# avik-pal/RegNeuralDE.jl

Hardware: AMD Instinct MI355X
Metric: training-step samples/sec + mean NFE, MNIST Neural ODE bs=512 (higher is better)
Workload: dtype f32; 1 GPU; MNIST NODE regularized (error_est), Tsit5 reltol=abstol=1.4e-8, batch 512 per GPU, 1xMI355X per rank; step = loss fwd + reverse pass through the solver + InvDecay/Momentum update; the weights train during the timed steps (mean_nfe drifts with --steps: value_fixed_weights of --full is the stationary companion); global_batch=512, parallelism=single

## Files before the change

### regneuralde.jl_amd/csrc/rnde_reverse.hip

```cpp
#include "rnde_node.h"
#include "rnde_wgradx.h"

static rnde_status chain_bwd_run(rnde_node* h, const float* u_bar_dev, const float* saveval_bar_host, float* x_bar_dev,
                                 float* p_bar_dev, float* tspan_bar_host, hipStream_t s, bool sync = true, float* tspan_bar_dev = nullptr);
static rnde_status bwd_run(rnde_node* h, const float* u_bar_dev, const float* saveval_bar_host, float* x_bar_dev,
                           float* p_bar_dev, float* tspan_bar_host, hipStream_t s, bool sync = true, float* tspan_bar_dev = nullptr);


extern "C" rnde_status rnde_node_backward_async(rnde_node* h, const float* u_bar_dev, const float* saveval_bar_host, float* x_bar_dev,
                                                float* p_bar_dev, float* tspan_bar_dev, void* stream) {
    if (!h) return RNDE_ERR_BAD_ARG;
    if (!h->have_tape) { h->err = "no recorded forward"; return RNDE_ERR_NO_TAPE; }
    if (h->engine == 3) return chain_bwd_run(h, u_bar_dev, saveval_bar_host, x_bar_dev, p_bar_dev, nullptr, (hipStream_t)stream, false, tspan_bar_dev);
    return bwd_run(h, u_bar_dev, saveval_bar_host, x_bar_dev, p_bar_dev, nullptr, (hipStream_t)stream, false, tspan_bar_dev);
}

extern "C" rnde_status rnde_node_backward(rnde_node* h, const float* u_bar_dev, const float* saveval_bar_host,
                                          float* x_bar_dev, float* p_bar_dev, float* tspan_bar_host, void* stream) {
    if (!h) return RNDE_ERR_BAD_ARG;
    if (!h->have_tape) { h->err = "no recorded forward"; return RNDE_ERR_NO_TAPE; }
    if (h->engine == 3) return chain_bwd_run(h, u_bar_dev, saveval_bar_host, x_bar_dev, p_bar_dev, tspan_bar_host, (hipStream_t)stream);
    return bwd_run(h, u_bar_dev, saveval_bar_host, x_bar_dev, p_bar_dev, tspan_bar_host, (hipStream_t)stream);
}
extern "C" rnde_status rnde_node_backward_host(rnde_node* h, const float* u_bar, const float* saveval_bar, float* x_bar,
                                               float* p_bar, float* tspan_bar) {
    if (!h) return RNDE_ERR_BAD_ARG;
    float *ub = nullptr, *xb = nullptr, *pb = nullptr;
    const size_t nb = (size_t)h->D * h->B * 4;
    HIPCHK(h, hipMalloc((void**)&ub, nb)); HIPCHK(h, hipMalloc((void**)&xb, nb)); HIPCHK(h, hipMalloc((void**)&pb, (size_t)h->P * 4));
    HIPCHK(h, hipMemcpy(ub, u_bar, nb, hipMemcpyHostToDevice));
    rnde_status st = rnde_node_backward(h, ub, saveval_bar, xb, pb, tspan_bar, nullptr);
    if (st == RNDE_OK) { hipMemcpy(x_bar, xb, nb, hipMemcpyDeviceToHost); hipMemcpy(p_bar, pb, (size_t)h->P * 4, hipMemcpyDeviceToHost); }
    hipFree(ub); hipFree(xb); hipFree(pb);
    return st;
}

static rnde_status bwd_prepare(rnde_node* h) {
    BwdBuffers& b = h->bw;
    if (b.ready) return RNDE_OK;
    const size_t A = (size_t)h->D * h->Bpad_max, HB = (size_t)h->H * h->Bpad_max;
    const int cap = h->cfg.max_attempts;
    HIPCHK(h, hipMalloc((void**)&b.U, A * 4)); HIPCHK(h, hipMalloc((void**)&b.K1, A * 4)); HIPCHK(h, hipMalloc((void**)&b.UB1, A * 4));
    HIPCHK(h, hipMalloc((void**)&b.zi2, 2 * A * 4)); HIPCHK(h, hipMalloc((void**)&b.zi1, 2 * HB * 4));
    HIPCHK(h, hipMalloc((void**)&b.svb_att, (size_t)cap * 4));
    HIPCHK(h, hipMalloc((void**)&b.bstate, 2 * sizeof(BState) + 64)); HIPCHK(h, hipMalloc((void**)&b.ibstate, 2 * sizeof(IBState)));
    HIPCHK(h, hipMalloc((void**)&b.bpart, (size_t)(2 * h->nwg_max + 256) * 4 * 4)); HIPCHK(h, hipMalloc((void**)&b.ipart, (size_t)2 * h->nwg_max * 4 * 4));
    HIPCHK(h, hipMalloc((void**)&b.tspan_out, 2 * 4));
    const size_t nev = (size_t)6 * cap + 2;
    const size_t desc_blob = 2 * nev * sizeof(EvalDesc) + (size_t)cap * 4 + 64;
    HIPCHK(h, hipMalloc((void**)&b.ev1, desc_blob)); HIPCHK(h, hipMalloc((void**)&b.ev2, nev * sizeof(EvalDesc)));
    HIPCHK(h, hipHostMalloc((void**)&b.h_ev1, desc_blob)); HIPCHK(h, hipHostMalloc((void**)&b.h_ev2, nev * sizeof(EvalDesc)));
    HIPCHK(h, hipHostMalloc((void**)&b.h_svb, (size_t)cap * 4));
    const size_t seg = std::max((size_t)h->H * (h->D + 2), (size_t)h->D * (h->H + 2));
    b.slab_floats = seg * 256;
    HIPCHK(h, hipMalloc((void**)&b.slab, 2 * b.slab_floats * 4));
    HIPCHK(h, hipMalloc((void**)&b.slab_r, 2 * 16 * seg * 4));
    if (!h->wstream) {
        int prio_least = 0, prio_greatest = 0;
        (void)hipDeviceGetStreamPriorityRange(&prio_least, &prio_greatest);
        HIPCHK(h, hipStreamCreateWithPriority(&h->wstream, hipStreamNonBlocking, prio_least));
        h->wevents.resize(66);
        for (auto& e : h->wevents) HIPCHK(h, hipEventCreateWithFlags(&e, hipEventDisableTiming));
    }
    if (h->engine == 2) {
        HIPCHK(h, hipMalloc((void**)&b.UTB, A * 4)); HIPCHK(h, hipMalloc((void**)&b.UNB, A * 4)); HIPCHK(h, hipMalloc((void**)&b.UPB0, A * 4));
        HIPCHK(h, hipMalloc((void**)&b.GB, 15 * A * 4));
    }
    b.ready = true;
    return RNDE_OK;
}

static bool wgrad3_ok(int M, int Nx) {
    const bool tall = M >= Nx;
    const int wide = tall ? M : Nx + 2, narrow = tall ? Nx + 2 : M;
    return getenv("RNDE_WGRAD_LEGACY") == nullptr && getenv("RNDE_WGRAD_V2") == nullptr && M % 4 == 0 && Nx % 4 == 0 && wide > 656 &&
           wide <= 800 && narrow <= 112;
}
static rnde_status launch_wgrad_part(rnde_node* h, const EvalDesc* ev, int n_evals, int per_chunk, int M, int Nx, int Bpad,
                                     float* slab, int* chunk_cursor, hipStream_t s, int max_chunks = 0) {
    if (n_evals <= 0) return RNDE_OK;
    const int mtiles = (M + 31) / 32, ntiles = (Nx + 2 + 31) / 32;
    const bool tall = M >= Nx;
    const int MB = tall ? 2 : 4, NB = tall ? 4 : 2;
    const int blocks = ((mtiles + MB - 1) / MB) * ((ntiles + NB - 1) / NB);
    const long long len = (long long)M * (Nx + 2);
    const int chunks = (n_evals + per_chunk - 1) / per_chunk;
    float* dst = slab + (size_t)(*chunk_cursor) * len;
    static const bool legacy = getenv("RNDE_WGRAD_LEGACY") != nullptr;
    const bool fits = tall ? (Nx + 2 <= 128) : (M <= 128);
    if (wgrad3_ok(M, Nx)) {
        const int total_steps = n_evals * ((Bpad + 31) / 32);
        static const int target_chunks = getenv("RNDE_WGRAD3_CHUNKS") ? atoi(getenv("RNDE_WGRAD3_CHUNKS")) : 128;
        int sc = std::max(1, std::min({max_chunks > 0 ? max_chunks : target_chunks, total_steps, 256}));
        const int steps_per_chunk = (total_steps + sc - 1) / sc;
        sc = (total_steps + steps_per_chunk - 1) / steps_per_chunk;
        if ((size_t)(*chunk_cursor + sc) * (size_t)len > h->bw.slab_floats) { h->err = "weight-gradient slab overflow"; return RNDE_ERR_BAD_ARG; }
        const bool x3_off = getenv("RNDE_X3_WGRAD_OFF") != nullptr;
        const bool x3_half = getenv("RNDE_X3_WGRAD_HALF") != nullptr;
        const int TT4 = ((tall ? M : Nx + 2) + 15) / 16;
        if (h->x3_packed && !x3_off && !x3_half && TT4 >= 28 && TT4 <= 52) {
            static const int target4 = getenv("RNDE_WGRAD4_CHUNKS") ? atoi(getenv("RNDE_WGRAD4_CHUNKS")) : 64;
            int sc4 = std::max(1, std::min({max_chunks > 0 ? max_chunks / 2 : target4, total_steps, 256}));
            const int spc4 = (total_steps + sc4 - 1) / sc4;
            sc4 = (total_steps + spc4 - 1) / spc4;
            if ((size_t)(*chunk_cursor + sc4) * (size_t)len > h->bw.slab_floats) { h->err = "weight-gradient slab overflow"; return RNDE_ERR_BAD_ARG; }
            static DeviceOnce attr4;
            if (attr4.need()) {
                HIPCHK(h, hipFuncSetAttribute((const void*)rnde_wgrad4x_kernel<true>, hipFuncAttributeMaxDynamicSharedMemorySize, (int)kWx4LdsBytes));
                HIPCHK(h, hipFuncSetAttribute((const void*)rnde_wgrad4x_kernel<false>, hipFuncAttributeMaxDynamicSharedMemorySize, (int)kWx4LdsBytes));
                attr4.done();
            }
            const dim3 g4(32 * ((sc4 + 7) / 8));
            if (tall) hipLaunchKernelGGL((rnde_wgrad4x_kernel<true>), g4, dim3(448), kWx4LdsBytes, s, ev, n_evals, spc4, sc4, M, Nx, Bpad, dst);
            else hipLaunchKernelGGL((rnde_wgrad4x_kernel<false>), g4, dim3(448), kWx4LdsBytes, s, ev, n_evals, spc4, sc4, M, Nx, Bpad, dst);
            HIPCHK(h, hipGetLastError());
            *chunk_cursor += sc4;
            return RNDE_OK;
        }
        if (h->x3_packed && !x3_off) {
            static DeviceOnce attrx;
            if (attrx.need()) {
                HIPCHK(h, hipFuncSetAttribute((const void*)rnde_wgrad3x_kernel<true>, hipFuncAttributeMaxDynamicSharedMemorySize, (int)kWxLdsBytes));
                HIPCHK(h, hipFuncSetAttribute((const void*)rnde_wgrad3x_kernel<false>, hipFuncAttributeMaxDynamicSharedMemorySize, (int)kWxLdsBytes));
                attrx.done();
            }
            if (tall) hipLaunchKernelGGL((rnde_wgrad3x_kernel<true>), dim3(2, sc), dim3(448), kWxLdsBytes, s, ev, n_evals, steps_per_chunk, M, Nx, Bpad, dst);
            else hipLaunchKernelGGL((rnde_wgrad3x_kernel<false>), dim3(2, sc), dim3(448), kWxLdsBytes, s, ev, n_evals, steps_per_chunk, M, Nx, Bpad, dst);
            HIPCHK(h, hipGetLastError());
            *chunk_cursor += sc;
            return RNDE_OK;
        }
        const size_t lds = (size_t)2 * 32 * (464 + 144) * sizeof(float);
        static DeviceOnce attr;
        if (attr.need()) {
            HIPCHK(h, hipFuncSetAttribute((const void*)rnde_wgrad3_kernel<true>, hipFuncAttributeMaxDynamicSharedMemorySize, (int)lds));
            HIPCHK(h, hipFuncSetAttribute((const void*)rnde_wgrad3_kernel<false>, hipFuncAttributeMaxDynamicSharedMemorySize, (int)lds));
            attr.done();
        }
        if (tall) hipLaunchKernelGGL((rnde_wgrad3_kernel<true>), dim3(2, sc), dim3(448), lds, s, ev, n_evals, steps_per_chunk, M, Nx, Bpad, dst);
        else hipLaunchKernelGGL((rnde_wgrad3_kernel<false>), dim3(2, sc), dim3(448), lds, s, ev, n_evals, steps_per_chunk, M, Nx, Bpad, dst);
        HIPCHK(h, hipGetLastError());
        *chunk_cursor += sc;
        return RNDE_OK;
    }
    if (!legacy && fits) {
        const int pblocks = tall ? (M + 127) / 128 : (Nx + 2 + 127) / 128;
        const int total_steps = n_evals * ((Bpad + 31) / 32);
        static const int target_wgs = getenv("RNDE_WGRAD_WGS") ? atoi(getenv("RNDE_WGRAD_WGS")) : 768;
        int sc = std::max(1, std::min({target_wgs / pblocks, total_steps, 256}));
        const int steps_per_chunk = (total_steps + sc - 1) / sc;
        sc = (total_steps + steps_per_chunk - 1) / steps_per_chunk;
        if ((size_t)(*chunk_cursor + sc) * (size_t)len > h->bw.slab_floats) { h->err = "weight-gradient slab overflow"; return RNDE_ERR_BAD_ARG; }
        if (tall) hipLaunchKernelGGL((rnde_wgrad2_kernel<true>), dim3(pblocks, sc), dim3(256), 0, s, ev, n_evals, steps_per_chunk, M, Nx, Bpad, dst);
        else hipLaunchKernelGGL((rnde_wgrad2_kernel<false>), dim3(pblocks, sc), dim3(256), 0, s, ev, n_evals, steps_per_chunk, M, Nx, Bpad, dst);
        HIPCHK(h, hipGetLastError());
        *chunk_cursor += sc;
        return RNDE_OK;
    } else {
        if ((size_t)(*chunk_cursor + chunks) * (size_t)len > h->bw.slab_floats) { h->err = "weight-gradient slab overflow"; return RNDE_ERR_BAD_ARG; }
        if (tall) hipLaunchKernelGGL((rnde_wgrad_kernel<2, 4>), dim3(blocks, chunks), dim3(64), 0, s, ev, n_evals, per_chunk, M, Nx, Bpad, dst);
        else hipLaunchKernelGGL((rnde_wgrad_kernel<4, 2>), dim3(blocks, chunks), dim3(64), 0, s, ev, n_evals, per_chunk, M, Nx, Bpad, dst);
    }
    HIPCHK(h, hipGetLastError());
    *chunk_cursor += chunks;
    return RNDE_OK;
}
static rnde_status launch_wgrad_reduce(rnde_node* h, const float* slab, int chunks, int M, int Nx, float* out, hipStream_t s) {
    const long long len = (long long)M * (Nx + 2);
    const int grid = (int)std::min<long long>((len + 255) / 256, 2048);
    if (chunks <= 16) {
        hipLaunchKernelGGL(rnde_wgrad_reduce, dim3(grid, 1), dim3(256), 0, s, slab, chunks, chunks, len, out);
    } else {
        const int per_group = (chunks + 15) / 16, groups = (chunks + per_group - 1) / per_group;
        hipLaunchKernelGGL(rnde_wgrad_reduce, dim3(grid, groups), dim3(256), 0, s, slab, chunks, per_group, len, h->bw.slab_r);
        hipLaunchKernelGGL(rnde_wgrad_reduce, dim3(grid, 1), dim3(256), 0, s, (const float*)h->bw.slab_r, groups, groups, len, out);
    }
    HIPCHK(h, hipGetLastError());
    return RNDE_OK;
}

static rnde_status bwd_run(rnde_node* h, const float* u_bar_dev, const float* saveval_bar_host, float* x_bar_dev,
                           float* p_bar_dev, float* tspan_bar_host, hipStream_t s, bool sync, float* tspan_bar_dev) {
    HIPCHK(h, hipSetDevice(h->cfg.device));
    rnde_status st = bwd_prepare(h);
    if (st != RNDE_OK) return st;
    BwdBuffers& b = h->bw;
    int n_att = h->n_att;
    const float svb_scale = h->couple ? (float)h->couple_world : 1.f;
    for (int i = 0; i < n_att; ++i)
        b.h_svb[i] = (saveval_bar_host && h->sv_index[i] >= 0) ? svb_scale * saveval_bar_host[h->sv_index[i]] : 0.f;
    const int ne_all = 2 + 6 * n_att;
    EvalDesc* const h_ev1 = b.h_ev1; EvalDesc* const h_ev2 = b.h_ev1 + ne_all; float* const h_svb_blob = (float*)(b.h_ev1 + 2 * (size_t)ne_all);
    EvalDesc* const d_ev1 = b.ev1;   EvalDesc* const d_ev2 = b.ev1 + ne_all;   float* const d_svb = (float*)(b.ev1 + 2 * (size_t)ne_all);
    memcpy(h_svb_blob, b.h_svb, (size_t)n_att * 4);
    BwdParams Q{};
    Q.F = make_params(h, h->xcopy, h->B, h->t0, h->t1, 1);
    Q.U = b.U; Q.K1 = b.K1; Q.UB1 = b.UB1; Q.zi2 = b.zi2; Q.zi1 = b.zi1; Q.svb_att = d_svb;
    Q.bstate = b.bstate; Q.ibstate = b.ibstate; Q.bpart = b.bpart; Q.ipart = b.ipart;
    Q.ubar = u_bar_dev; Q.xbar = x_bar_dev; Q.tspan_out = b.tspan_out;
    Q.n_att = n_att; Q.track_ctrl = h->cfg.track_ctrl; Q.track_initdt = h->cfg.track_initdt; Q.reg_kind = h->cfg.regularize;
    Q.bpart_n = Q.F.nwg;
    Q.tspan_scale = h->couple ? 1.f / (float)h->couple_world : 1.f;
#ifdef RNDE_DIAG
    if (getenv("RNDE_DIAG_BWD")) { if (!h->diag_buf) hipMalloc((void**)&h->diag_buf, 8192); hipMemset(h->diag_buf, 0, 512); Q.F.dbg_out = h->diag_buf; }
#endif
    Q.sv_T = (int)h->saveat.size();
    Q.sv_ubar0 = (!h->saveat.empty() && h->saveat[0] == h->t0) ? u_bar_dev : nullptr;
    if (!h->saveat.empty() && h->engine != 2) { h->err = "saveat reverse pass runs on the stage engine only"; return RNDE_ERR_BAD_ARG; }
    const long long A = (long long)h->D * Q.F.Bpad, HB = (long long)h->H * Q.F.Bpad;
    RecLayout L{A, HB};
    int ne = 2;
    h_ev2[0] = EvalDesc{b.zi2, h->h0, h->t0, 0};           h_ev1[0] = EvalDesc{b.zi1, h->xcopy, h->t0, 0};
    h_ev2[1] = EvalDesc{b.zi2 + A, h->h1, h->t0 + h->h_init->dt0, 0}; h_ev1[1] = EvalDesc{b.zi1 + HB, h->u1, h->t0 + h->h_init->dt0, 0};
    for (int n = 0; n < n_att; ++n) {
        const StepMeta& m = h->h_meta[n];
        const float* R = h->arena + (long long)m.rec * h->rec_stride;
        for (int sidx = 2; sidx <= 7; ++sidx) {
            const float ts = m.t + tsC(sidx - 1) * m.dt;
            h_ev2[ne] = EvalDesc{R + L.k(sidx), R + L.h(sidx), ts, 0};
            h_ev1[ne] = EvalDesc{R + L.z1(sidx), sidx < 7 ? R + L.g(sidx) : R + L.unew(), ts, 0};
            ++ne;
        }
    }
    HIPCHK(h, hipMemcpyAsync(b.ev1, b.h_ev1, 2 * (size_t)ne * sizeof(EvalDesc) + (size_t)n_att * 4, hipMemcpyHostToDevice, s));
    float* slab1 = b.slab;
    float* slab2w = b.slab + b.slab_floats;
    int cur1 = 0, cur2 = 0, evi = 0;
    const int per_chunk = std::max(1, (ne + 239) / 240);
    const int side_pct = h->wgrad_side_pct;
    const int sweep_cus = 8 * h->sR * ((Q.F.Bpad / 16 + 7) / 8);
    const bool side = h->engine == 2 && h->persist == 1 && side_pct > 0 && n_att >= 8 && sweep_cus <= 224 &&
                      wgrad3_ok(h->H, h->D) && wgrad3_ok(h->D, h->H);
    const int side_att = side ? std::min(n_att, n_att * side_pct / 100) : 0;
    const int group = std::max(4, (side_att + 5) / 6);
    bool used_side = false;
    auto wgrad_group = [&](int lo, int hi, bool on_side) -> rnde_status {
        if (hi <= lo) return RNDE_OK;
        hipStream_t ws = s;
        if (on_side) {
            hipEvent_t ev = h->wevents[evi++ % 64];
            HIPCHK(h, hipEventRecord(ev, s));
            HIPCHK(h, hipStreamWaitEvent(h->wstream, ev, 0));
            ws = h->wstream; used_side = true;
        }
        rnde_status r = launch_wgrad_part(h, d_ev1 + lo, hi - lo, per_chunk, h->H, h->D, h->B, slab1, &cur1, ws, on_side ? 16 : 0);
        if (r != RNDE_OK) return r;
        return launch_wgrad_part(h, d_ev2 + lo, hi - lo, per_chunk, h->D, h->H, h->B, slab2w, &cur2, ws, on_side ? 16 : 0);
    };
    int hi_att = n_att;
    hipError_t e;
    h->tev_bwd = false;
    if (h->timing) HIPCHK(h, hipEventRecord(h->tev[2], s));
    if (h->engine == 2) {
        if (!h->rev_packed) {
            HIPCHK(h, stage_pack(h, h->pcopy, h->spwBt, 2, h->sMT, h->sKHb, s));
            HIPCHK(h, stage_pack(h, h->pcopy, h->spwDt, 3, h->sHT, h->sMT, s));
        }
        h->rev_packed = false;
        BStageParams BQ{};
        BQ.B = Q; BQ.p = h->pcopy; BQ.pwBt = h->spwBt; BQ.pwDt = h->spwDt; BQ.slab = h->slab2; BQ.x3Bt = h->x3Bt; BQ.x3Dt = h->x3Dt;
        BQ.UTB = b.UTB; BQ.UNB = b.UNB; BQ.UPB0 = b.UPB0; BQ.GB = b.GB;
        BQ.EXK = b.GB + 6 * A; BQ.EXG = b.GB + 7 * A; BQ.SVW = b.GB + 8 * A;
        BQ.sv_t = h->saveat.empty() ? nullptr : h->sv_t_dev; BQ.sv_ubar = u_bar_dev; BQ.nsave = (int)h->saveat.size();
        BQ.MT = h->sMT; BQ.WT = h->sWT; BQ.R = h->sR; BQ.C = Q.F.Bpad / 16; BQ.HT = h->sHT; BQ.KHb = h->sKHb;
        double* const bsum = (double*)(b.bstate + 2);
        const bool pre_reduce = h->persist == 1 && Q.bpart_n >= 896 && !getenv("RNDE_NO_BPART_REDUCE");
        if (pre_reduce) BQ.B.bsum = bsum;
        const dim3 grid(BQ.R * BQ.C), blk(64 * BQ.WT);
        std::vector<int> sv_lo(n_att, 0), sv_hi(n_att, 0);
        if (!h->saveat.empty()) {
            int ns = (h->saveat[0] == h->t0) ? 1 : 0;
            for (int n = 0; n < n_att; ++n) {
                sv_lo[n] = ns;
                if (h->h_meta[n].flags & F_ACCEPT) {
                    const float tnew = h->h_meta[n].t + h->h_meta[n].dt;
                    while (ns < (int)h->saveat.size() && h->saveat[ns] <= tnew) ++ns;
                }
                sv_hi[n] = ns;
            }
        }
        auto eig_coefs = [&](int n, float& c1, float& c2) {
            c1 = 0.f; c2 = 0.f;
            const StepMeta& mm = h->h_meta[n];
            const bool eg_ok = !(mm.eigen == 0.f || mm.eigen != mm.eigen);
            double eigb = 0.0;
            if (h->cfg.regularize == RNDE_REG_STIFF && eg_ok) eigb = (double)b.h_svb[n] * (mm.eigen > 0 ? 1.0 : -1.0) / 3.5068;
            if (h->cfg.regularize == RNDE_REG_ERR_STIFF && eg_ok) eigb = 0.1 * (double)b.h_svb[n] / 3.5068;
            if (h->cfg.regularize == RNDE_REG_STIFF_DT && eg_ok) eigb = (double)b.h_svb[n] * ((double)mm.eigen * (double)mm.dt > 0 ? 1.0 : -1.0) * (double)mm.dt;
            if (eigb != 0.0 && mm.n1 > 0.f && mm.n2 > 0.f) {
                c1 = (float)(eigb / ((double)mm.n2 * (double)mm.n1));
                c2 = (float)(-eigb * ((double)mm.n1 / (double)mm.n2) / ((double)mm.n2 * (double)mm.n2));
            }
        };
        for (int n = n_att - 1; n >= 0; --n) {
            float c1 = 0.f, c2 = 0.f;
            eig_coefs(n, c1, c2);
            const double qo = pow((double)h->h_meta[n].qold_in, (double)kBeta2);
            if (h->persist == 1) {
                PersistSync Y{h->tslab, h->pabort, h->pxcc, h->persist_spins};
                HIPCHK(h, slab_prepare(h, Q.F.Bpad, s));
                const dim3 pgrid(8 * BQ.R * ((BQ.C + 7) / 8));
                const bool fix = BQ.WT == 7 && BQ.HT == 7 && BQ.KHb == 7 && BQ.MT == 49 && BQ.R == 7 && h->D == 784 && h->H == 100 && !h->stage_generic;
                if (fix) {
                    const size_t flds = h->stage_lds + (size_t)(RNDE_BSTAGE_HDMA ? 1 : 0) * 6 * 7 * 2 * 1024;
                    static DeviceOnce attr;
                    if (attr.need()) {
                        HIPCHK(h, hipFuncSetAttribute((const void*)rnde_bstage_attempt_kernel<1, 1>, hipFuncAttributeMaxDynamicSharedMemorySize, 160 * 1024));
                        HIPCHK(h, hipFuncSetAttribute((const void*)rnde_bstage_attempt_kernel<0, 1>, hipFuncAttributeMaxDynamicSharedMemorySize, 160 * 1024));
                        attr.done();
                    }
                    const bool x3 = h->x3_packed && h->x3Bt && h->x3Dt && !getenv("RNDE_X3_REV_OFF");
                    if (x3) {
                        const size_t xlds = sizeof(float) * ((size_t)2 * kX3ImageFloats + 64) + (size_t)(RNDE_BSTAGE_HDMA ? 1 : 0) * 6 * 7 * 2 * 1024;
                        static DeviceOnce attr3;
                        if (attr3.need()) {
#define RNDE_X3_ATTR(A, E) HIPCHK(h, hipFuncSetAttribute((const void*)rnde_bstage_attempt_kernel<A, 1, 1, E>, hipFuncAttributeMaxDynamicSharedMemorySize, 160 * 1024));
                            RNDE_X3_ATTR(1, 0) RNDE_X3_ATTR(1, 1) RNDE_X3_ATTR(1, 2) RNDE_X3_ATTR(1, 3) RNDE_X3_ATTR(0, 0) RNDE_X3_ATTR(0, 1) RNDE_X3_ATTR(0, 2) RNDE_X3_ATTR(0, 3)
#undef RNDE_X3_ATTR
                            attr3.done();
                        }
                        const int ex = (h->saveat.empty() ? 0 : 1) | (h->cfg.regularize >= RNDE_REG_STIFF ? 2 : 0);
#define RNDE_X3_LAUNCH(A, E) hipLaunchKernelGGL((rnde_bstage_attempt_kernel<A, 1, 1, E>), pgrid, blk, xlds, s, BQ, n, h->h_meta[n], c1, c2, sv_lo[n], sv_hi[n], Y, qo, b.h_svb[n])
                        if (h->act2) { if (ex == 0) RNDE_X3_LAUNCH(1, 0); else if (ex == 1) RNDE_X3_LAUNCH(1, 1); else if (ex == 2) RNDE_X3_LAUNCH(1, 2); else RNDE_X3_LAUNCH(1, 3); }
                        else { if (ex == 0) RNDE_X3_LAUNCH(0, 0); else if (ex == 1) RNDE_X3_LAUNCH(0, 1); else if (ex == 2) RNDE_X3_LAUNCH(0, 2); else RNDE_X3_LAUNCH(0, 3); }
#undef RNDE_X3_LAUNCH
                    } else if (h->act2) hipLaunchKernelGGL((rnde_bstage_attempt_kernel<1, 1>), pgrid, blk, flds, s, BQ, n, h->h_meta[n], c1, c2, sv_lo[n], sv_hi[n], Y, qo, b.h_svb[n]);
                    else hipLaunchKernelGGL((rnde_bstage_attempt_kernel<0, 1>), pgrid, blk, flds, s, BQ, n, h->h_meta[n], c1, c2, sv_lo[n], sv_hi[n], Y, qo, b.h_svb[n]);
                } else if (h->act2) hipLaunchKernelGGL((rnde_bstage_attempt_kernel<1, 0>), pgrid, blk, h->stage_lds, s, BQ, n, h->h_meta[n], c1, c2, sv_lo[n], sv_hi[n], Y, qo, b.h_svb[n]);
                else hipLaunchKernelGGL((rnde_bstage_attempt_kernel<0, 0>), pgrid, blk, h->stage_lds, s, BQ, n, h->h_meta[n], c1, c2, sv_lo[n], sv_hi[n], Y, qo, b.h_svb[n]);
                if ((st = couple_sum(h, b.bpart + (size_t)(n & 1) * Q.bpart_n * 4, 4LL * Q.bpart_n, s)) != RNDE_OK) return st;
                if (pre_reduce && n > 0) hipLaunchKernelGGL(rnde_bpart_reduce_kernel, dim3(1), dim3(64), 0, s, Q, n, bsum);
                if (n >= n_att - side_att && (hi_att - n >= group || n == n_att - side_att)) {
                    st = wgrad_group(2 + 6 * n, 2 + 6 * hi_att, true);
                    if (st != RNDE_OK) return st;
                    hi_att = n;
                }
                continue;
            }
            if (h->act2) hipLaunchKernelGGL((rnde_bstage_kernel<1, BM_START>), grid, blk, h->stage_lds, s, BQ, n, 0, h->h_meta[n], c1, c2, sv_lo[n], sv_hi[n], qo);
            else hipLaunchKernelGGL((rnde_bstage_kernel<0, BM_START>), grid, blk, h->stage_lds, s, BQ, n, 0, h->h_meta[n], c1, c2, sv_lo[n], sv_hi[n], qo);
            for (int j = 6; j >= 1; --j) {
                if (h->act2) hipLaunchKernelGGL((rnde_bstage_kernel<1, BM_STAGE>), grid, blk, h->stage_lds, s, BQ, n, j, h->h_meta[n], c1, c2, sv_lo[n], sv_hi[n], qo);
                else hipLaunchKernelGGL((rnde_bstage_kernel<0, BM_STAGE>), grid, blk, h->stage_lds, s, BQ, n, j, h->h_meta[n], c1, c2, sv_lo[n], sv_hi[n], qo);
            }
            if ((st = couple_sum(h, b.bpart + (size_t)(n & 1) * Q.bpart_n * 4, 4LL * Q.bpart_n, s)) != RNDE_OK) return st;
        }
        HIPCHK(h, hipGetLastError());
        {
            if (h->act2) {
                hipLaunchKernelGGL((rnde_binit_stage_kernel<1, 0>), grid, blk, h->stage_lds, s, BQ);
                hipLaunchKernelGGL((rnde_binit_stage_kernel<1, 1>), grid, blk, h->stage_lds, s, BQ);
            } else {
                hipLaunchKernelGGL((rnde_binit_stage_kernel<0, 0>), grid, blk, h->stage_lds, s, BQ);
                hipLaunchKernelGGL((rnde_binit_stage_kernel<0, 1>), grid, blk, h->stage_lds, s, BQ);
            }
            if ((st = couple_sum(h, Q.ipart, 4LL * Q.F.nwg, s)) != RNDE_OK) return st;
            if (h->act2) {
                hipLaunchKernelGGL((rnde_binit_stage_kernel<1, 2>), grid, blk, h->stage_lds, s, BQ);
                hipLaunchKernelGGL((rnde_binit_stage_kernel<1, 3>), grid, blk, h->stage_lds, s, BQ);
            } else {
                hipLaunchKernelGGL((rnde_binit_stage_kernel<0, 2>), grid, blk, h->stage_lds, s, BQ);
                hipLaunchKernelGGL((rnde_binit_stage_kernel<0, 3>), grid, blk, h->stage_lds, s, BQ);
            }
            if ((st = couple_sum(h, Q.ipart + 4LL * Q.F.nwg, 4LL * Q.F.nwg, s)) != RNDE_OK) return st;
            hipLaunchKernelGGL(rnde_bfin_kernel, dim3(1), dim3(64), 0, s, Q);
            HIPCHK(h, hipGetLastError());
        }
    }
    if (h->timing) HIPCHK(h, hipEventRecord(h->tev[3], s));
    st = wgrad_group(0, 2 + 6 * hi_att, false);
    if (st != RNDE_OK) return st;
    if (used_side) {
        hipEvent_t ev = h->wevents[64];
        HIPCHK(h, hipEventRecord(ev, h->wstream));
        HIPCHK(h, hipStreamWaitEvent(s, ev, 0));
    }
    if (cur1 > 16 && cur2 > 16) {
        const long long len1 = (long long)h->H * (h->D + 2), len2 = (long long)h->D * (h->H + 2);
        const size_t seg_r = std::max((size_t)len1, (size_t)len2);
        float* r1 = b.slab_r; float* r2 = b.slab_r + 16 * seg_r;
        const int pg1 = (cur1 + 15) / 16, g1 = (cur1 + pg1 - 1) / pg1, pg2 = (cur2 + 15) / 16, g2 = (cur2 + pg2 - 1) / pg2;
        const int grid = (int)std::min<long long>((std::max(len1, len2) + 255) / 256, 2048);
        ReducePair A{{{slab1, r1, len1, cur1, pg1}, {slab2w, r2, len2, cur2, pg2}}};
        hipLaunchKernelGGL(rnde_wgrad_reduce_pair, dim3(grid, std::max(g1, g2), 2), dim3(256), 0, s, A);
        ReducePair Bp{{{r1, p_bar_dev, len1, g1, g1}, {r2, p_bar_dev + (size_t)h->H * (h->D + 2), len2, g2, g2}}};
        hipLaunchKernelGGL(rnde_wgrad_reduce_pair, dim3(grid, 1, 2), dim3(256), 0, s, Bp);
        HIPCHK(h, hipGetLastError());
    } else {
        st = launch_wgrad_reduce(h, slab1, cur1, h->H, h->D, p_bar_dev, s);
        if (st != RNDE_OK) return st;
        st = launch_wgrad_reduce(h, slab2w, cur2, h->D, h->H, p_bar_dev + (size_t)h->H * (h->D + 2), s);
        if (st != RNDE_OK) return st;
    }
    if (h->timing) { HIPCHK(h, hipEventRecord(h->tev[4], s)); h->tev_bwd = true; }
#ifdef RNDE_DIAG
    if (h->engine == 2 && h->persist == 1 && getenv("RNDE_DIAG_BWD")) {
        unsigned long long hst[64] = {0};
        hipStreamSynchronize(s);
        hipMemcpy(hst, h->diag_buf, sizeof(hst), hipMemcpyDeviceToHost);
        fprintf(stderr, "persistent reverse attempt (workgroup 0 thread 0, cycles): START %lld (entry->weights issued %lld, ->w1t %lld, ->array loads issued %lld, finish_attempt_scalars %lld, scalar chain %lld, vector part %lld), its phase D + put %lld\n", (long long)(hst[1]-hst[0]), (long long)(hst[43]-hst[0]), (long long)(hst[44]-hst[43]), (long long)(hst[40]-hst[44]), (long long)(hst[41]-hst[40]), (long long)(hst[42]-hst[41]), (long long)(hst[1]-hst[42]), (long long)(hst[2]-hst[1]));
        for (int st = 0; st < 6; ++st) { const unsigned long long* q = hst + 3 + 5 * st; const unsigned long long prev = st == 0 ? hst[2] : hst[7 + 5 * (st - 1)];
            fprintf(stderr, "  stage j=%d: poll %lld A %lld B %lld C %lld D+put %lld\n", 6 - st, (long long)(q[0]-prev), (long long)(q[1]-q[0]), (long long)(q[2]-q[1]), (long long)(q[3]-q[2]), st < 5 ? (long long)(q[4]-q[3]) : 0LL); }
        fprintf(stderr, "  total %lld cycles to the end of stage 1, END (reduction of the 21 partial sums) %lld; in START's vector part the wait for the record's k arrays %lld\n",
                (long long)(hst[34]-hst[0]), (long long)(hst[35]-hst[34]), (long long)(hst[45]-hst[42]));
    }
#endif
    if (!sync) {
        if (tspan_bar_dev) HIPCHK(h, hipMemcpyAsync(tspan_bar_dev, b.tspan_out, 8, hipMemcpyDeviceToDevice, s));
        h->have_tape = false;
        h->pending_bwd = (h->engine == 2 && h->persist == 1);
        return RNDE_OK;
    }
    HIPCHK(h, hipMemcpyAsync(h->h_scal, b.tspan_out, 8, hipMemcpyDeviceToHost, s));
    if (h->engine == 2) persist_check_enqueue(h, h->sR * (Q.F.Bpad / 16), s);
    HIPCHK(h, hipStreamSynchronize(s));
    if (h->couple && rnde_comm_health(h->couple) != RNDE_OK) { h->err = std::string("coupled controller: ") + rnde_comm_last_error(h->couple); return RNDE_ERR_HIP; }
    if (tspan_bar_host) { tspan_bar_host[0] = h->h_scal[0]; tspan_bar_host[1] = h->h_scal[1]; }
// ... 406 lines not shown
```

### regneuralde.jl_amd/csrc/rnde_wgradx.h

```cpp
#pragma once
#include "rnde_x3.h"

namespace rnde {

constexpr int kWxRowShorts = 40;
constexpr int kWxTallRows = 400, kWxNarrowRows = 112;
constexpr int kWxPlaneShortsT = kWxTallRows * kWxRowShorts, kWxPlaneShortsS = kWxNarrowRows * kWxRowShorts;
constexpr size_t kWxLdsBytes = (size_t)3 * (kWxPlaneShortsT + kWxPlaneShortsS) * 2;

template <bool TALL_IS_Z>
__global__ __launch_bounds__(448) void rnde_wgrad3x_kernel(const EvalDesc* __restrict__ evals, int n_evals, int per_chunk, int M, int Nx, int Bpad, float* __restrict__ slab) {
    constexpr int KC = 32;
    extern __shared__ __attribute__((aligned(16))) unsigned short wxs[];
    unsigned short* TP = wxs;
    unsigned short* SP = wxs + 3 * kWxPlaneShortsT;
    const int tid = threadIdx.x, lane = tid & 63, w = __builtin_amdgcn_readfirstlane(tid >> 6);
    const int mrow = lane & 15, kk = lane >> 4;
    const int TR = TALL_IS_Z ? M : Nx + 2, SR = TALL_IS_Z ? Nx + 2 : M;
    const int TRp = TALL_IS_Z ? M : Nx, SRp = TALL_IS_Z ? Nx : M;
    const int TT = (TR + 15) >> 4, T0 = (TT + 1) >> 1;
    const int half = blockIdx.x, chunk = blockIdx.y;
    const int tile_lo = half ? T0 : 0, tile_hi = half ? TT : T0, ntile = tile_hi - tile_lo;
    const int row_lo = 16 * tile_lo, nrow = 16 * ntile;
    const int steps_per_eval = (Bpad + KC - 1) / KC;
    const int s_lo = chunk * per_chunk, s_hi = min(n_evals * steps_per_eval, s_lo + per_chunk);
    const int total_steps = max(0, s_hi - s_lo);
    x3f4 acc[4][7];
#pragma unroll
    for (int i = 0; i < 4; ++i)
#pragma unroll
        for (int n = 0; n < 7; ++n) acc[i][n] = (x3f4){0.f, 0.f, 0.f, 0.f};
    const bool has3 = w + 21 < ntile;

    constexpr unsigned kNoSrc = 0x7FFFFF00u;
    int u_kind[5], u_dst[5];
    unsigned u_voff[5];
#pragma unroll
    for (int jj = 0; jj < 4; ++jj) {
        const int u = tid + 448 * jj;
        int kind = 0, dst = 0; unsigned voff = kNoSrc;
        if (u < 4 * nrow) {
            const int o = u / nrow, row = u - o * nrow, gr = row_lo + row;
            kind = gr < TRp ? 1 : (!TALL_IS_Z && gr == TRp ? 2 : (!TALL_IS_Z && gr == TRp + 1 ? 3 : 4));
            if (kind == 1) voff = 4u * (unsigned)(gr + 8 * o * TRp);
            dst = row * kWxRowShorts + 8 * o;
        }
        u_kind[jj] = kind; u_voff[jj] = voff; u_dst[jj] = dst;
    }
    {
        const int o = tid / kWxNarrowRows, row = tid - o * kWxNarrowRows;
        const int kind = row < SRp ? 1 : (TALL_IS_Z && row == SRp ? 2 : (TALL_IS_Z && row == SRp + 1 ? 3 : 4));
        u_kind[4] = kind; u_voff[4] = kind == 1 ? 4u * (unsigned)(row + 8 * o * SRp) : kNoSrc;
        u_dst[4] = 3 * kWxPlaneShortsT + row * kWxRowShorts + 8 * o;
    }
    int e_nx = s_lo / steps_per_eval, cs_nx = s_lo - e_nx * steps_per_eval;
    float stg[5][8];
    float stg_t = 0.f; int stg_ncols = 0;
    auto fetch = [&]() {
        const int e = e_nx, c0 = cs_nx * KC;
        if (++cs_nx == steps_per_eval) { cs_nx = 0; ++e_nx; }
        stg_t = evals[e].t;
        stg_ncols = min(KC, Bpad - c0);
        __amdgpu_buffer_rsrc_t rsT = __builtin_amdgcn_make_buffer_rsrc((void*)(TALL_IS_Z ? evals[e].Z : evals[e].X), 0, 4 * TRp * Bpad, 0x00020000);
        __amdgpu_buffer_rsrc_t rsS = __builtin_amdgcn_make_buffer_rsrc((void*)(TALL_IS_Z ? evals[e].X : evals[e].Z), 0, 4 * SRp * Bpad, 0x00020000);
#pragma unroll
        for (int jj = 0; jj < 5; ++jj) {
            const int cs = jj < 4 ? TRp : SRp;
#pragma unroll
            for (int j = 0; j < 8; ++j) {
                const unsigned off = u_voff[jj] + 4u * (unsigned)((c0 + j) * cs);
                stg[jj][j] = __builtin_bit_cast(float, __builtin_amdgcn_raw_buffer_load_b32(jj < 4 ? rsT : rsS, (int)off, 0, 2));
            }
        }
    };
    auto spill = [&]() {
#pragma unroll
        for (int jj = 0; jj < 5; ++jj) {
            const int kind = u_kind[jj];
            if (kind == 0) continue;
            const int o8 = u_dst[jj] % kWxRowShorts;
            float v[8];
#pragma unroll
            for (int j = 0; j < 8; ++j) v[j] = kind == 1 ? stg[jj][j] : ((kind == 2 || kind == 3) && o8 + j < stg_ncols ? (kind == 2 ? stg_t : 1.f) : 0.f);
            unsigned hi[4], mid[4], lo[4];
#pragma unroll
            for (int j = 0; j < 4; ++j) x3_split2(v[2 * j], v[2 * j + 1], hi[j], mid[j], lo[j]);
            unsigned short* d = wxs + u_dst[jj];
            const int ps = jj < 4 ? kWxPlaneShortsT : kWxPlaneShortsS;
            *(x3u4*)d = (x3u4){hi[0], hi[1], hi[2], hi[3]};
            *(x3u4*)(d + ps) = (x3u4){mid[0], mid[1], mid[2], mid[3]};
            *(x3u4*)(d + 2 * ps) = (x3u4){lo[0], lo[1], lo[2], lo[3]};
        }
    };
    auto fragT = [&](int tile, int pl) { return *(const x3u4*)(TP + pl * kWxPlaneShortsT + (16 * tile + mrow) * kWxRowShorts + 8 * kk); };
    auto fragS = [&](int tile, int pl) { return *(const x3u4*)(SP + pl * kWxPlaneShortsS + (16 * tile + mrow) * kWxRowShorts + 8 * kk); };

    if (total_steps > 0) { fetch(); spill(); }
    __syncthreads();
    for (int step = 0; step < total_steps; ++step) {
        if (step + 1 < total_steps) fetch();
#pragma unroll
        for (int ps = 0; ps < 2; ++ps) {
            x3u4 a[2][3];
#pragma unroll
            for (int i = 0; i < 2; ++i) {
                const int ii = 2 * ps + i, tile = (ii < 3 || has3) ? w + 7 * ii : w;
#pragma unroll
                for (int pl = 0; pl < 3; ++pl) a[i][pl] = fragT(tile, pl);
            }
#pragma unroll
            for (int n = 0; n < 7; ++n) {
                __builtin_amdgcn_sched_barrier(0);
                const x3u4 bh = fragS(n, 0), bm = fragS(n, 1), bl = fragS(n, 2);
#define WX_TERM(PA, BV) _Pragma("unroll") for (int i = 0; i < 2; ++i) if (2 * ps + i < 3 || has3) acc[2 * ps + i][n] = x3_mfma(a[i][PA], BV, acc[2 * ps + i][n]);
                WX_TERM(2, bh) WX_TERM(0, bl) WX_TERM(1, bm) WX_TERM(1, bh) WX_TERM(0, bm) WX_TERM(0, bh)
#undef WX_TERM
            }
        }
        __syncthreads();
        if (step + 1 < total_steps) spill();
        __syncthreads();
    }
    float* out = slab + (size_t)chunk * M * (Nx + 2);
#pragma unroll
    for (int i = 0; i < 4; ++i) {
        if (w + 7 * i < ntile) {
#pragma unroll
            for (int n = 0; n < 7; ++n) {
                const int sr = 16 * n + mrow;
#pragma unroll
                for (int q = 0; q < 4; ++q) {
                    const int tr = row_lo + 16 * (w + 7 * i) + 4 * kk + q;
                    if (tr < TR && sr < SR) out[TALL_IS_Z ? (size_t)sr * M + tr : (size_t)tr * M + sr] = acc[i][n][q];
                }
            }
        }
    }
}

#ifndef RNDE_WX4_SB
#define RNDE_WX4_SB 1
#endif
#ifndef RNDE_WX4_ABL
#define RNDE_WX4_ABL 0
#endif
constexpr int kWx4TallRows = 208;
constexpr int kWx4PlaneT = kWx4TallRows * kWxRowShorts, kWx4PlaneS = kWxNarrowRows * kWxRowShorts;
constexpr int kWx4ImageShorts = 3 * (kWx4PlaneT + kWx4PlaneS);
constexpr size_t kWx4LdsBytes = (size_t)2 * kWx4ImageShorts * 2;

template <bool TALL_IS_Z>
__global__ __launch_bounds__(448) void rnde_wgrad4x_kernel(const EvalDesc* __restrict__ evals, int n_evals, int per_chunk, int n_chunks, int M, int Nx, int Bpad,
                                                           float* __restrict__ slab) {
    constexpr int KC = 32;
    extern __shared__ __attribute__((aligned(16))) unsigned short wxs[];
    const int tid = threadIdx.x, lane = tid & 63, w = __builtin_amdgcn_readfirstlane(tid >> 6);
    const int mrow = lane & 15, kk = lane >> 4;
    const int lin = blockIdx.x, xcd = lin & 7, within = lin >> 3;
    const int chunk = (within >> 2) * 8 + xcd, part = within & 3;
    if (chunk >= n_chunks) return;
    const int TR = TALL_IS_Z ? M : Nx + 2, SR = TALL_IS_Z ? Nx + 2 : M;
    const int TRp = TALL_IS_Z ? M : Nx, SRp = TALL_IS_Z ? Nx : M;
    const int TT = (TR + 15) >> 4, base = TT >> 2, rem = TT & 3;
    const int ntile = base + (part < rem ? 1 : 0), tile_lo = part * base + (part < rem ? part : rem);
    const int row_lo = 16 * tile_lo, nrow = 16 * ntile;
    const int steps_per_eval = (Bpad + KC - 1) / KC;
    const int s_lo = chunk * per_chunk, s_hi = min(n_evals * steps_per_eval, s_lo + per_chunk);
    const int total_steps = max(0, s_hi - s_lo);
    x3f4 acc[2][7];
#pragma unroll
    for (int i = 0; i < 2; ++i)
#pragma unroll
        for (int n = 0; n < 7; ++n) acc[i][n] = (x3f4){0.f, 0.f, 0.f, 0.f};
    const bool has2 = w + 7 < ntile;
    const int tile1 = has2 ? w + 7 : w;

    constexpr unsigned kNoSrc = 0x7FFFFF00u;
    const bool wide_wave = w < 4;
    const int Rp = wide_wave ? TRp : SRp;
    const int nunit = wide_wave ? nrow : kWxNarrowRows;
    const int uid = (wide_wave ? tid : tid - 256) % nunit;
    const int uq = uid >> 2, uo = uid & 3;
    const int u_gr = (wide_wave ? row_lo : 0) + 4 * uq;
    const bool u_mem = u_gr < Rp;
    const bool u_syn = u_gr == Rp && (wide_wave ? !TALL_IS_Z : TALL_IS_Z);
    const float syn_f = u_syn ? 1.f : 0.f;
    const unsigned u_voff = u_mem ? 4u * (unsigned)(u_gr + 8 * uo * Rp) : kNoSrc;
    const int u_dst = (wide_wave ? 0 : 3 * kWx4PlaneT) + 4 * uq * kWxRowShorts + 8 * uo;
    const int u_ps = wide_wave ? kWx4PlaneT : kWx4PlaneS;
    int e_nx = s_lo / steps_per_eval, cs_nx = s_lo - e_nx * steps_per_eval, left = total_steps;
    x3f4 stg[2][8];
    float stg_t[2] = {0.f, 0.f}; int stg_ncols[2] = {0, 0};
    auto fetch = [&](auto set_c) {
        constexpr int SET = decltype(set_c)::value;
        const int e = e_nx, c0 = cs_nx * KC;
        {
            const bool adv = --left > 0, wrap = cs_nx + 1 == steps_per_eval;
            e_nx = (adv && wrap) ? e_nx + 1 : e_nx;
            cs_nx = adv ? (wrap ? 0 : cs_nx + 1) : cs_nx;
        }
        stg_t[SET] = evals[e].t;
        stg_ncols[SET] = min(KC, Bpad - c0);
        const float* src = wide_wave == TALL_IS_Z ? evals[e].Z : evals[e].X;
        __amdgpu_buffer_rsrc_t rs = __builtin_amdgcn_make_buffer_rsrc((void*)src, 0, 4 * Rp * Bpad, 0x00020000);
#pragma unroll
        for (int j = 0; j < 8; ++j)
            stg[SET][j] = __builtin_bit_cast(x3f4, __builtin_amdgcn_raw_buffer_load_b128(rs, (int)u_voff, 4 * (c0 + j) * Rp, 0));
    };
    unsigned abl_sink = 0u;
    auto spill_row = [&](unsigned short* img, int i, auto set_c) {
        constexpr int SET = decltype(set_c)::value;
        float v[8];
#pragma unroll
        for (int j = 0; j < 8; ++j) v[j] = i < 2 ? stg[SET][j][i] + (i == 0 ? syn_f * stg_t[SET] : syn_f) : stg[SET][j][i];
        unsigned hi[4], mid[4], lo[4];
#if RNDE_WX4_ABL == 6
#pragma unroll
        for (int j = 0; j < 4; ++j) { hi[j] = __float_as_uint(v[2 * j]); mid[j] = __float_as_uint(v[2 * j + 1]); lo[j] = hi[j]; }
#else
#pragma unroll
        for (int j = 0; j < 4; ++j) x3_split2(v[2 * j], v[2 * j + 1], hi[j], mid[j], lo[j]);
#endif
        unsigned short* d = img + u_dst + i * kWxRowShorts;
#if RNDE_WX4_ABL == 5
        abl_sink ^= hi[0] ^ hi[1] ^ hi[2] ^ hi[3] ^ mid[0] ^ mid[1] ^ mid[2] ^ mid[3] ^ lo[0] ^ lo[1] ^ lo[2] ^ lo[3];
        (void)d;
#else
        *(x3u4*)d = (x3u4){hi[0], hi[1], hi[2], hi[3]};
        *(x3u4*)(d + u_ps) = (x3u4){mid[0], mid[1], mid[2], mid[3]};
        *(x3u4*)(d + 2 * u_ps) = (x3u4){lo[0], lo[1], lo[2], lo[3]};
#endif
    };
    unsigned short* const img0 = wxs;
    unsigned short* const img1 = wxs + kWx4ImageShorts;
    if (total_steps == 0) return;
    typedef std::integral_constant<int, 0> S0;
    typedef std::integral_constant<int, 1> S1;
    fetch(S0{});
#pragma unroll
    for (int i = 0; i < 4; ++i) spill_row(img0, i, S0{});
    fetch(S0{});
    fetch(S1{});
    __syncthreads();
    auto one_step = [&](const unsigned short* cur, unsigned short* nxt, auto more_c, auto set_c) {
        constexpr bool MORE = decltype(more_c)::value;
        const unsigned short* SPc = cur + 3 * kWx4PlaneT;
        auto fragT = [&](int tile, int pl) { return *(const x3u4*)(cur + pl * kWx4PlaneT + (16 * tile + mrow) * kWxRowShorts + 8 * kk); };
        auto fragS = [&](int tile, int pl) { return *(const x3u4*)(SPc + pl * kWx4PlaneS + (16 * tile + mrow) * kWxRowShorts + 8 * kk); };
        x3u4 a[2][3];
#pragma unroll
        for (int pl = 0; pl < 3; ++pl) { a[0][pl] = fragT(w, pl); a[1][pl] = fragT(tile1, pl); }
        x3u4 bh = fragS(0, 0), bm = fragS(0, 1), bl = fragS(0, 2);
#pragma unroll
        for (int n = 0; n < 7; ++n) {
            x3u4 nh = bh, nm = bm, nl = bl;
#if RNDE_WX4_ABL != 3 && RNDE_WX4_ABL != 4
            if (n < 6) { nh = fragS(n + 1, 0); nm = fragS(n + 1, 1); nl = fragS(n + 1, 2); }
#endif
#if RNDE_WX4_ABL != 1 && RNDE_WX4_ABL != 2 && RNDE_WX4_ABL != 4
            if (MORE && n < 4) spill_row(nxt, n, set_c);
#endif
#if RNDE_WX4_ABL != 2 && RNDE_WX4_ABL != 4
            if (MORE && n == 4) fetch(set_c);
#endif
#define WX4_TERM(PA, BV) { acc[0][n] = x3_mfma(a[0][PA], BV, acc[0][n]); acc[1][n] = x3_mfma(a[1][PA], BV, acc[1][n]); }
            WX4_TERM(2, bh) WX4_TERM(0, bl) WX4_TERM(1, bm) WX4_TERM(1, bh) WX4_TERM(0, bm) WX4_TERM(0, bh)
#undef WX4_TERM
            bh = nh; bm = nm; bl = nl;
#if RNDE_WX4_SB
            __builtin_amdgcn_sched_barrier(0);
#endif
        }
    };
    int step = 0;
    for (; step + 2 < total_steps; step += 2) {
        one_step(img0, img1, std::true_type{}, S0{});
        __syncthreads();
        one_step(img1, img0, std::true_type{}, S1{});
        __syncthreads();
    }
    if (total_steps - step == 2) {
        one_step(img0, img1, std::true_type{}, S0{});
        __syncthreads();
        one_step(img1, nullptr, std::false_type{}, S1{});
    } else one_step(img0, nullptr, std::false_type{}, S0{});
#if RNDE_WX4_ABL == 5
    if (abl_sink == 0x12345678u) slab[0] = 1.f;
#endif
    float* out = slab + (size_t)chunk * M * (Nx + 2);
#pragma unroll
    for (int i = 0; i < 2; ++i) {
        if (w + 7 * i < ntile) {
#pragma unroll
            for (int n = 0; n < 7; ++n) {
                const int sr = 16 * n + mrow;
#pragma unroll
                for (int q = 0; q < 4; ++q) {
                    const int tr = row_lo + 16 * (w + 7 * i) + 4 * kk + q;
                    if (tr < TR && sr < SR) out[TALL_IS_Z ? (size_t)sr * M + tr : (size_t)tr * M + sr] = acc[i][n][q];
                }
            }
        }
    }
}

}
```

Before: 306,300 samples/s.

## Use quad-fast LDS image layout and lane-streamed staging in wgrad4x kernel

```diff
diff --git a/regneuralde.jl_amd/csrc/rnde_reverse.hip b/regneuralde.jl_amd/csrc/rnde_reverse.hip
--- a/regneuralde.jl_amd/csrc/rnde_reverse.hip
+++ b/regneuralde.jl_amd/csrc/rnde_reverse.hip
@@ -106,13 +106,21 @@
             if ((size_t)(*chunk_cursor + sc4) * (size_t)len > h->bw.slab_floats) { h->err = "weight-gradient slab overflow"; return RNDE_ERR_BAD_ARG; }
             static DeviceOnce attr4;
             if (attr4.need()) {
-                HIPCHK(h, hipFuncSetAttribute((const void*)rnde_wgrad4x_kernel<true>, hipFuncAttributeMaxDynamicSharedMemorySize, (int)kWx4LdsBytes));
-                HIPCHK(h, hipFuncSetAttribute((const void*)rnde_wgrad4x_kernel<false>, hipFuncAttributeMaxDynamicSharedMemorySize, (int)kWx4LdsBytes));
+                HIPCHK(h, hipFuncSetAttribute((const void*)rnde_wgrad4x_kernel<true, true>, hipFuncAttributeMaxDynamicSharedMemorySize, (int)kWx4sLdsBytes));
+                HIPCHK(h, hipFuncSetAttribute((const void*)rnde_wgrad4x_kernel<false, true>, hipFuncAttributeMaxDynamicSharedMemorySize, (int)kWx4sLdsBytes));
+                HIPCHK(h, hipFuncSetAttribute((const void*)rnde_wgrad4x_kernel<true, false>, hipFuncAttributeMaxDynamicSharedMemorySize, (int)kWx4LdsBytes));
+                HIPCHK(h, hipFuncSetAttribute((const void*)rnde_wgrad4x_kernel<false, false>, hipFuncAttributeMaxDynamicSharedMemorySize, (int)kWx4LdsBytes));
                 attr4.done();
             }
             const dim3 g4(32 * ((sc4 + 7) / 8));
-            if (tall) hipLaunchKernelGGL((rnde_wgrad4x_kernel<true>), g4, dim3(448), kWx4LdsBytes, s, ev, n_evals, spc4, sc4, M, Nx, Bpad, dst);
-            else hipLaunchKernelGGL((rnde_wgrad4x_kernel<false>), g4, dim3(448), kWx4LdsBytes, s, ev, n_evals, spc4, sc4, M, Nx, Bpad, dst);
+            const bool segments = getenv("RNDE_X3_WGRAD_SEGMENTS") != nullptr;
+            if (segments) {
+                if (tall) hipLaunchKernelGGL((rnde_wgrad4x_kernel<true, false>), g4, dim3(448), kWx4LdsBytes, s, ev, n_evals, spc4, sc4, M, Nx, Bpad, dst);
+                else hipLaunchKernelGGL((rnde_wgrad4x_kernel<false, false>), g4, dim3(448), kWx4LdsBytes, s, ev, n_evals, spc4, sc4, M, Nx, Bpad, dst);
+            } else {
+                if (tall) hipLaunchKernelGGL((rnde_wgrad4x_kernel<true, true>), g4, dim3(448), kWx4sLdsBytes, s, ev, n_evals, spc4, sc4, M, Nx, Bpad, dst);
+                else hipLaunchKernelGGL((rnde_wgrad4x_kernel<false, true>), g4, dim3(448), kWx4sLdsBytes, s, ev, n_evals, spc4, sc4, M, Nx, Bpad, dst);
+            }
             HIPCHK(h, hipGetLastError());
             *chunk_cursor += sc4;
             return RNDE_OK;
diff --git a/regneuralde.jl_amd/csrc/rnde_wgradx.h b/regneuralde.jl_amd/csrc/rnde_wgradx.h
--- a/regneuralde.jl_amd/csrc/rnde_wgradx.h
+++ b/regneuralde.jl_amd/csrc/rnde_wgradx.h
@@ -148,11 +148,17 @@
 constexpr int kWx4PlaneT = kWx4TallRows * kWxRowShorts, kWx4PlaneS = kWxNarrowRows * kWxRowShorts;
 constexpr int kWx4ImageShorts = 3 * (kWx4PlaneT + kWx4PlaneS);
 constexpr size_t kWx4LdsBytes = (size_t)2 * kWx4ImageShorts * 2;
-
-template <bool TALL_IS_Z>
+constexpr int kWx4sQT = kWx4TallRows / 4, kWx4sQS = kWxNarrowRows / 4;
+static_assert(kWx4sQT % 8 == 4 && kWx4sQS % 8 == 4, "the quad-fast image is conflict-free for ds_read_b128 only with Q = 4 mod 8");
+constexpr int kWx4sPlaneT = 16 * kWx4sQT * 8, kWx4sPlaneS = 16 * kWx4sQS * 8;
+constexpr int kWx4sImageShorts = 3 * (kWx4sPlaneT + kWx4sPlaneS);
+constexpr size_t kWx4sLdsBytes = (size_t)2 * kWx4sImageShorts * 2;
+
+template <bool TALL_IS_Z, bool STREAM>
 __global__ __launch_bounds__(448) void rnde_wgrad4x_kernel(const EvalDesc* __restrict__ evals, int n_evals, int per_chunk, int n_chunks, int M, int Nx, int Bpad,
                                                            float* __restrict__ slab) {
     constexpr int KC = 32;
+    constexpr int PlaneT = STREAM ? kWx4sPlaneT : kWx4PlaneT, PlaneS = STREAM ? kWx4sPlaneS : kWx4PlaneS, ImageShorts = STREAM ? kWx4sImageShorts : kWx4ImageShorts;
     extern __shared__ __attribute__((aligned(16))) unsigned short wxs[];
     const int tid = threadIdx.x, lane = tid & 63, w = __builtin_amdgcn_readfirstlane(tid >> 6);
     const int mrow = lane & 15, kk = lane >> 4;
@@ -162,7 +168,7 @@
     const int TR = TALL_IS_Z ? M : Nx + 2, SR = TALL_IS_Z ? Nx + 2 : M;
     const int TRp = TALL_IS_Z ? M : Nx, SRp = TALL_IS_Z ? Nx : M;
     const int TT = (TR + 15) >> 4, base = TT >> 2, rem = TT & 3;
-    const int ntile = base + (part < rem ? 1 : 0), tile_lo = part * base + (part < rem ? part : rem);
+    const int ntile = base + ((STREAM ? part >= 4 - rem : part < rem) ? 1 : 0), tile_lo = part * base + (STREAM ? max(0, part - (4 - rem)) : (part < rem ? part : rem));
     const int row_lo = 16 * tile_lo, nrow = 16 * ntile;
     const int steps_per_eval = (Bpad + KC - 1) / KC;
     const int s_lo = chunk * per_chunk, s_hi = min(n_evals * steps_per_eval, s_lo + per_chunk);
@@ -179,21 +185,34 @@
     const bool wide_wave = w < 4;
     const int Rp = wide_wave ? TRp : SRp;
     const int nunit = wide_wave ? nrow : kWxNarrowRows;
-    const int uid = (wide_wave ? tid : tid - 256) % nunit;
-    const int uq = uid >> 2, uo = uid & 3;
+    int uq, uo;
+    if (STREAM) {
+        const int nq = nunit >> 2, l = wide_wave ? lane : lane & 31;
+        uq = l < nq ? l : (l - 16 < nq && wide_wave ? l - 16 : (l - 8 < nq ? l - 8 : l % nq));
+        uo = wide_wave ? w : 2 * ((w - 4) & 1) + (lane >> 5);
+    } else {
+        const int uid = (wide_wave ? tid : tid - 256) % nunit;
+        uq = uid >> 2; uo = uid & 3;
+    }
     const int u_gr = (wide_wave ? row_lo : 0) + 4 * uq;
     const bool u_mem = u_gr < Rp;
     const bool u_syn = u_gr == Rp && (wide_wave ? !TALL_IS_Z : TALL_IS_Z);
     const float syn_f = u_syn ? 1.f : 0.f;
     const unsigned u_voff = u_mem ? 4u * (unsigned)(u_gr + 8 * uo * Rp) : kNoSrc;
-    const int u_dst = (wide_wave ? 0 : 3 * kWx4PlaneT) + 4 * uq * kWxRowShorts + 8 * uo;
-    const int u_ps = wide_wave ? kWx4PlaneT : kWx4PlaneS;
+    const int u_Q = wide_wave ? kWx4sQT : kWx4sQS;
+    const int u_dst = (wide_wave ? 0 : 3 * PlaneT) + (STREAM ? 8 * (4 * uo * u_Q + uq) : 4 * uq * kWxRowShorts + 8 * uo);
+    const int u_ps = wide_wave ? PlaneT : PlaneS;
+    const int u_rs = STREAM ? 8 * u_Q : kWxRowShorts;
     int e_nx = s_lo / steps_per_eval, cs_nx = s_lo - e_nx * steps_per_eval, left = total_steps;
     x3f4 stg[2][8];
     float stg_t[2] = {0.f, 0.f}; int stg_ncols[2] = {0, 0};
     auto fetch = [&](auto set_c) {
         constexpr int SET = decltype(set_c)::value;
+#if RNDE_WX4_ABL == 7
+        const int e = s_lo / steps_per_eval, c0 = (s_lo - e * steps_per_eval) * KC;
+#else
         const int e = e_nx, c0 = cs_nx * KC;
+#endif
         {
             const bool adv = --left > 0, wrap = cs_nx + 1 == steps_per_eval;
             e_nx = (adv && wrap) ? e_nx + 1 : e_nx;
@@ -221,7 +240,7 @@
 #pragma unroll
         for (int j = 0; j < 4; ++j) x3_split2(v[2 * j], v[2 * j + 1], hi[j], mid[j], lo[j]);
 #endif
-        unsigned short* d = img + u_dst + i * kWxRowShorts;
+        unsigned short* d = img + u_dst + i * u_rs;
 #if RNDE_WX4_ABL == 5
         abl_sink ^= hi[0] ^ hi[1] ^ hi[2] ^ hi[3] ^ mid[0] ^ mid[1] ^ mid[2] ^ mid[3] ^ lo[0] ^ lo[1] ^ lo[2] ^ lo[3];
         (void)d;
@@ -232,7 +251,7 @@
 #endif
     };
     unsigned short* const img0 = wxs;
-    unsigned short* const img1 = wxs + kWx4ImageShorts;
+    unsigned short* const img1 = wxs + ImageShorts;
     if (total_steps == 0) return;
     typedef std::integral_constant<int, 0> S0;
     typedef std::integral_constant<int, 1> S1;
@@ -244,9 +263,13 @@
     __syncthreads();
     auto one_step = [&](const unsigned short* cur, unsigned short* nxt, auto more_c, auto set_c) {
         constexpr bool MORE = decltype(more_c)::value;
-        const unsigned short* SPc = cur + 3 * kWx4PlaneT;
-        auto fragT = [&](int tile, int pl) { return *(const x3u4*)(cur + pl * kWx4PlaneT + (16 * tile + mrow) * kWxRowShorts + 8 * kk); };
-        auto fragS = [&](int tile, int pl) { return *(const x3u4*)(SPc + pl * kWx4PlaneS + (16 * tile + mrow) * kWxRowShorts + 8 * kk); };
+        const unsigned short* SPc = cur + 3 * PlaneT;
+        auto fragT = [&](int tile, int pl) {
+            return *(const x3u4*)(cur + pl * PlaneT + (STREAM ? 8 * ((4 * kk + (mrow & 3)) * kWx4sQT + 4 * tile + (mrow >> 2)) : (16 * tile + mrow) * kWxRowShorts + 8 * kk));
+        };
+        auto fragS = [&](int tile, int pl) {
+            return *(const x3u4*)(SPc + pl * PlaneS + (STREAM ? 8 * ((4 * kk + (mrow & 3)) * kWx4sQS + 4 * tile + (mrow >> 2)) : (16 * tile + mrow) * kWxRowShorts + 8 * kk));
+        };
         x3u4 a[2][3];
 #pragma unroll
         for (int pl = 0; pl < 3; ++pl) { a[0][pl] = fragT(w, pl); a[1][pl] = fragT(tile1, pl); }
```

After: 310,500 samples/s (median of 6 runs). 1.01x the previous value.
